# MITIBMxGraph/SALIENT_plusplus

Hardware: AMD Instinct MI355X
Metric: sampled_edges_per_sec (higher is better)
Workload: dtype int64/fp16-copy

## Files before the change

salient_plusplus_amd/csrc/sampler.hip:

```cpp
#include "spp_internal.h"

#include <hipcub/hipcub.hpp>

#include <algorithm>
#include <chrono>
#include <cstdlib>
#include <cstring>
#include <vector>

#include <map>
#include <memory>
#include <mutex>
#include <tuple>

#include "fp8_body.hip.h"
#include "gather_body.hip.h"
#include "partition_common.hip.h"

#ifndef SPP_TILE_NT
#define SPP_TILE_NT 1024
#endif
#include "mt19937.hip.h"
#include "sampler_internal.h"

// ... 788 lines not shown
  for (int u = 0; u < kScatterEPT; ++u) {
    const int64_t p = base + u * kTileNT + threadIdx.x;
    v[u] = cval[p < pcap ? p : pcap - 1];
  }
  if (base >= E || err0) return;
  bool ok[kScatterEPT];
#pragma unroll
  for (int u = 0; u < kScatterEPT; ++u) {
    ok[u] = base + u * kTileNT + threadIdx.x < E;
    v[u] = (int32_t)((uint32_t)v[u] & idmask);
  }
  for (int b = threadIdx.x; b < nbk; b += kTileNT) cur[b] = 0;
  __syncthreads();
#pragma unroll
  for (int u = 0; u < kScatterEPT; ++u)
    if (ok[u]) atomicAdd(&cur[bucket_of((uint32_t)v[u], cb_log2)], 1);
  __syncthreads();
  {
    const int per = (nbk + kTileNT - 1) / kTileNT;
    const int b0 = threadIdx.x * per;
    int32_t c[kMaxBuckets / kTileNT], sum = 0;
#pragma unroll
    for (int k = 0; k < kMaxBuckets / kTileNT; ++k) {
      c[k] = (k < per && b0 + k < nbk) ? cur[b0 + k] : 0;
      sum += c[k];
    }
    int32_t tot;
    int32_t off = block_exclusive_scan<int32_t, kTileNT>(sum, lscan, &tot);
#pragma unroll
    for (int k = 0; k < kMaxBuckets / kTileNT; ++k) {
      if (k < per && b0 + k < nbk) {
        const int32_t g = c[k] ? __hip_atomic_fetch_add(bfill + b0 + k, c[k], __ATOMIC_RELAXED, __HIP_MEMORY_SCOPE_AGENT) : 0;
        cur[b0 + k] = off;
        delta[b0 + k] = g - off;
        off += c[k];
      }
    }
  }
  __syncthreads();
#pragma unroll
  for (int u = 0; u < kScatterEPT; ++u) {
    if (!ok[u]) continue;
    const uint32_t c = (uint32_t)v[u];
    const uint32_t b = bucket_of(c, cb_log2);
    const int32_t slot = atomicAdd(&cur[b], 1);
    const int32_t li = u * kTileNT + threadIdx.x;
    snode[slot] = c;
    sidx[slot] = (uint16_t)li;
    const int32_t rel = slot + delta[b];
    if (rel < bcap) {
      if (!tiled) inv[base + li] = (uint32_t)((int32_t)b * bcap + rel);
    } else {
      const int32_t j = __hip_atomic_fetch_add(G(s.ovfc) + h, 1, __ATOMIC_RELAXED, __HIP_MEMORY_SCOPE_AGENT);
      inv[base + (tiled ? slot : li)] = (uint32_t)(region + j);
      bpairs[(int64_t)region + j] = ((unsigned long long)c << 32) | (uint32_t)(base + li);
    }
  }
  __syncthreads();
  const int32_t n_tile = (int32_t)((E - base) < kScatterTile ? (E - base) : kScatterTile);
  SPP_GLOBAL uint16_t* tidx = G(s.tidx);
  for (int k = threadIdx.x; k < n_tile; k += kTileNT) {
    const uint32_t c = snode[k];
    const int32_t b = (int32_t)bucket_of(c, cb_log2);
    const int32_t rel = k + delta[b];
    if (rel < bcap) {
      bpairs[(int64_t)b * bcap + rel] = ((unsigned long long)c << 32) | (uint32_t)(base + sidx[k]);
      if (tiled) inv[base + k] = (uint32_t)(b * bcap + rel);
    }
    if (tiled) tidx[base + k] = sidx[k];
  }
}

__device__ __forceinline__ int32_t first_rank(const SlotPtrs& s, uint32_t q) {
  const uint32_t w = q >> 6;
  const RankWord rw = s.fwords[w];
  return s.fsum[q >> 8] + (int32_t)rw.pre + __popcll(rw.bits & ((1ull << (q & 63)) - 1ull));
}

template <int NS, bool kFlat = false>
__global__ __launch_bounds__(kNT) __attribute__((amdgpu_waves_per_eu(NS <= 3072 ? 6 : 1))) void k_bucket_dedup(const SlotPtrs* __restrict__ slots, GroupGrid gg,
                                                       int32_t hop_word, DedupGeom g, int32_t bcap, int32_t region) {
  SPP_GROUP_BLOCK(gg);
  const int32_t h = hop_word & 0xff, cb_log2 = (hop_word >> 8) & 0xff, hop_flags = hop_word >> 16;
  const int32_t last_hop = hop_flags & 1;
  const bool no_preread = hop_flags & 2;
  __shared__ unsigned long long tab[NS];
  __shared__ int32_t fkc[kMaxFinePerCoarse];
  __shared__ int32_t fnew[kMaxFinePerCoarse];
  __shared__ int ovf;
  const SlotPtrs& s = slots[gg.first_slot + by_];
  const SPP_GLOBAL SlotState* st = G(s.st);
  const SPP_GLOBAL unsigned long long* bpairs = G(s.bpairs);
  SPP_GLOBAL unsigned long long* known = G(s.known);
  SPP_GLOBAL int32_t* kcount = G(s.kcount);
  const SPP_GLOBAL RankWord* fwords = G(s.fwords);
  const SPP_GLOBAL int32_t* fsum = G(s.fsum);
  SPP_GLOBAL uint32_t* res = G(s.res);
  const int32_t b = bx_;
  const int32_t shift = g.nb_log2 - cb_log2;
  const int32_t nf = 1 << shift;
  const int32_t fb0 = b << shift;
  const int32_t err0 = st->error;
  const uint32_t T = (uint32_t)st->cnt[h];
  const uint32_t Tprev = h > 0 ? (uint32_t)st->cnt[h - 1] : 0u;
  const int32_t fill = __builtin_amdgcn_readfirstlane(G(s.bfill)[b]);
  const int32_t e0 = b * bcap, e1 = e0 + (fill < bcap ? fill : bcap);
  const bool spill = fill > bcap;
  for (int i = threadIdx.x; i < nf; i += kNT) {
    fkc[i] = kcount[fb0 + i];
    fnew[i] = 0;
  }
  const int lane = threadIdx.x & (kWave - 1);
  unsigned long long kpre[4];
  if constexpr (!kFlat) {
    const int lf0 = threadIdx.x / kWave;
    const SPP_GLOBAL unsigned long long* kl0 = known + (int64_t)(fb0 + (lf0 < nf ? lf0 : 0)) * g.kcap;
#pragma unroll
    for (int u = 0; u < 4; ++u) kpre[u] = kl0[lane + u * kWave];
  }
  if (err0) return;
  const bool work = e1 > e0;
  unsigned long long pr[kDedupRegs];
#pragma unroll
  for (int u = 0; u < kDedupRegs; ++u) {
    const int i = e0 + u * kNT + threadIdx.x;
    const unsigned long long v = bpairs[i < e1 ? i : 0];
    pr[u] = i < e1 ? v : kEmptySlot;
  }
  if (work)
    for (int i = threadIdx.x; i < NS; i += kNT) tab[i] = kEmptySlot;
  if (threadIdx.x == 0) ovf = 0;
  __syncthreads();
  if constexpr (kFlat) {
    __shared__ int32_t fpre[kMaxFinePerCoarse + 1];
    if (threadIdx.x < kWave) {
      const int32_t c = (int)threadIdx.x < nf ? fkc[threadIdx.x] : 0;
      const int32_t inc = wave_inclusive_scan(c);
      if ((int)threadIdx.x < nf) fpre[threadIdx.x + 1] = inc;
      if (threadIdx.x == 0) fpre[0] = 0;
    }
    __syncthreads();
    const int32_t K = fpre[nf];
    for (int j0 = threadIdx.x; j0 < K; j0 += 4 * kNT) {
      unsigned long long e[4];
      uint32_t q[4];
      RankWord rw[4];
      int32_t fs[4];
      SPP_GLOBAL unsigned long long* at[4];
#pragma unroll
      for (int u = 0; u < 4; ++u) {
// ... 55 lines not shown
        const bool pend = e[u] != kEmptySlot && (val & kPending);
        q[u] = pend ? (val & ~kPending) : 0u;
        rw[u] = load_rank_word(fwords, q[u] >> 6);
        fs[u] = fsum[q[u] >> 8];
      }
#pragma unroll
      for (int u = 0; u < 4; ++u) {
        if (e[u] == kEmptySlot) continue;
        uint32_t val = (uint32_t)e[u];
        if (val & kPending) {
          val = Tprev + (uint32_t)(fs[u] + (int32_t)rw[u].pre + __popcll(rw[u].bits & ((1ull << (q[u] & 63)) - 1ull)));
          e[u] = (e[u] & 0xffffffff00000000ull) | val;
          kl[i0 + u * kWave] = e[u];
        }
        if (work) lds_upsert<true, NS, false>(tab, (uint32_t)(e[u] >> 32), val, &ovf);
      }
    }
  }
  if (!work) return;
  __syncthreads();
#pragma unroll
  for (int u = 0; u < kDedupRegs; ++u)
    if (pr[u] != kEmptySlot) {
      if (no_preread) lds_upsert<false, NS, false>(tab, (uint32_t)(pr[u] >> 32), T + (uint32_t)pr[u], &ovf);
      else lds_upsert<false, NS>(tab, (uint32_t)(pr[u] >> 32), T + (uint32_t)pr[u], &ovf);
    }
  for (int i0 = e0 + kDedupRegs * kNT + threadIdx.x; i0 < e1; i0 += 4 * kNT) {
    unsigned long long q[4];
#pragma unroll
    for (int u = 0; u < 4; ++u) {
      const int i = i0 + u * kNT;
      const unsigned long long v = bpairs[i < e1 ? i : e0];
      q[u] = i < e1 ? v : kEmptySlot;
    }
#pragma unroll
    for (int u = 0; u < 4; ++u)
      if (q[u] != kEmptySlot) lds_upsert<false, NS, false>(tab, (uint32_t)(q[u] >> 32), T + (uint32_t)q[u], &ovf);
  }
  if (spill) {
    const int32_t n_ovf = G(s.ovfc)[h];
    for (int i = threadIdx.x; i < n_ovf; i += kNT) {
      const unsigned long long q = bpairs[(int64_t)region + i];
      if ((int32_t)bucket_of((uint32_t)(q >> 32), cb_log2) == b) lds_upsert<false, NS, false>(tab, (uint32_t)(q >> 32), T + (uint32_t)q, &ovf);
    }
  }
  __syncthreads();
  if (ovf) {
    if (threadIdx.x == 0) atomicOr(&s.st->error, kErrBucketCap);
    return;
  }
  auto resolve = [&](unsigned long long pair, int i) {
    const uint32_t key = (uint32_t)(pair >> 32), p = (uint32_t)pair;
    const uint32_t val = lds_find<NS>(tab, key);
    res[i] = val;
    if (val == T + p && !last_hop) {
      const int32_t lf = (int32_t)bucket_of(key, g.nb_log2) - fb0;
      const int j = fkc[lf] + atomicAdd(&fnew[lf], 1);
      if (j < g.kcap) known[(int64_t)(fb0 + lf) * g.kcap + j] = ((unsigned long long)key << 32) | kPending | p;
      else ovf = 1;
    }
  };
#pragma unroll
  for (int u = 0; u < kDedupRegs; ++u)
    if (pr[u] != kEmptySlot) resolve(pr[u], e0 + u * kNT + threadIdx.x);
  for (int i = e0 + kDedupRegs * kNT + threadIdx.x; i < e1; i += kNT) resolve(bpairs[i], i);
  if (spill) {
    const int32_t n_ovf = G(s.ovfc)[h];
    for (int i = threadIdx.x; i < n_ovf; i += kNT) {
      const unsigned long long q = bpairs[(int64_t)region + i];
      if ((int32_t)bucket_of((uint32_t)(q >> 32), cb_log2) == b) resolve(q, region + i);
    }
  }
  __syncthreads();
  if (threadIdx.x == 0) G(s.bfill)[b] = 0;
  if (threadIdx.x == 0 && ovf) atomicOr(&s.st->error, kErrBucketCap);
  for (int i = threadIdx.x; i < nf; i += kNT) {
    const int32_t room = g.kcap - fkc[i];
    kcount[fb0 + i] = fkc[i] + (fnew[i] < room ? fnew[i] : room);
  }
}

constexpr int kFlagNT = kNT;
#ifndef SPP_FLAG_ROUNDS
#define SPP_FLAG_ROUNDS 4
#endif
constexpr int kFlagRounds = SPP_FLAG_ROUNDS;
constexpr int kFlagSpan = kFlagNT * kFlagRounds;
static_assert(kFlagNT == 256, "a round of the workgroup is one rank block");

__device__ int32_t scan_block_sums_acquire(int32_t* a, int32_t n, int32_t* lds) {
  int32_t carry = 0;
  for (int32_t base = 0; base < n; base += kFlagNT) {
    const int32_t i = base + threadIdx.x;
    const int32_t v = (i < n) ? acquire_i32(&a[i]) : 0;
    int32_t tot;
    const int32_t ex = block_exclusive_scan<int32_t, kFlagNT>(v, lds, &tot);
    if (i < n) a[i] = carry + ex;
    carry += tot;
    __syncthreads();
  }
  return carry;
}

__global__ __launch_bounds__(kFlagNT) void k_hop_flag(const SlotPtrs* __restrict__ slots, GroupGrid gg, int32_t h,
                                                       int32_t f, int32_t ucap, int64_t pcap) {
  SPP_GROUP_BLOCK(gg);
  __shared__ int32_t wcnt[kFlagRounds][kFlagNT / kWave];
  __shared__ int32_t lscan[kFlagNT / kWave + 1];
  __shared__ int is_last;
  const SlotPtrs& s = slots[gg.first_slot + by_];
  SPP_GLOBAL SlotState* st = G(s.st);
  const SPP_GLOBAL uint32_t* inv = G(s.inv);
  const SPP_GLOBAL uint32_t* res = G(s.res);
  SPP_GLOBAL uint32_t* evals = G(s.evals);
  const int64_t base = (int64_t)bx_ * kFlagSpan;
  const int32_t err0 = st->error;
  const int32_t E = st->E[h];
  const uint32_t T = (uint32_t)st->cnt[h];
  uint32_t slot[kFlagRounds];
#pragma unroll
  for (int r = 0; r < kFlagRounds; ++r) {
    const int64_t p = base + r * kFlagNT + threadIdx.x;
    slot[r] = inv[p < pcap ? p : pcap - 1];
  }
  if (err0) {
    if (bx_ == 0 && threadIdx.x == 0) {
      st->cnt[h + 1] = (int32_t)T;
      st->dbase[h + 1] = st->dbase[h];
    }
    return;
  }
  const int32_t nwg = E > 0 ? (E + kFlagSpan - 1) / kFlagSpan : 1;
  if ((int32_t)bx_ >= nwg) return;
  const int wid = threadIdx.x / kWave, lane = threadIdx.x & (kWave - 1);
  uint32_t val[kFlagRounds];
#pragma unroll
  for (int r = 0; r < kFlagRounds; ++r) {
    const int64_t p = base + r * kFlagNT + threadIdx.x;
    val[r] = res[p < E ? slot[r] : 0u];
  }
  unsigned long long bits[kFlagRounds];
#pragma unroll
  for (int r = 0; r < kFlagRounds; ++r) {
    const int64_t p = base + r * kFlagNT + threadIdx.x;
    bool flag = false;
    if (p < E) {
      evals[p] = val[r];
      flag = (val[r] == T + (uint32_t)p);
    }
    bits[r] = __ballot(flag);
    if (lane == 0) wcnt[r][wid] = __popcll(bits[r]);
  }
  __syncthreads();
  if (lane == 0) {
#pragma unroll
    for (int r = 0; r < kFlagRounds; ++r) {
      int32_t pre = 0;
      for (int k = 0; k < wid; ++k) pre += wcnt[r][k];
      const int64_t blk = (int64_t)bx_ * kFlagRounds + r;
      s.fwords[blk * (kFlagNT / kWave) + wid] = RankWord{bits[r], (uint32_t)pre, 0u};
      if (wid == kFlagNT / kWave - 1)
        __hip_atomic_store(&s.fsum[blk], pre + wcnt[r][wid], __ATOMIC_RELAXED, __HIP_MEMORY_SCOPE_AGENT);
    }
  }
  asm volatile("s_waitcnt vmcnt(0)" ::: "memory");
  __syncthreads();
  if (threadIdx.x == 0) is_last = take_ticket_is_last(s.ctr, nwg) ? 1 : 0;
  __syncthreads();
  if (!is_last) return;
  const int32_t nblk = (E + 255) / 256;
  const int32_t nnew = scan_block_sums_acquire(s.fsum, nblk, lscan);
  if (threadIdx.x == 0) {
    const int32_t U = st->cnt[h] + nnew;
    st->cnt[h + 1] = U;
    st->dbase[h + 1] = st->dbase[h] + (int64_t)(f > 0 ? f : 0) * st->nsmp[h];
    if (U > ucap) atomicOr(&s.st->error, kErrNodeCap);
  }
}

constexpr int kFlagTileRounds = kScatterTile / kFlagNT;
__global__ __launch_bounds__(kFlagNT) void k_hop_flag_tiled(const SlotPtrs* __restrict__ slots, GroupGrid gg, int32_t h,
                                                             int32_t f, int32_t ucap, int64_t pcap) {
  SPP_GROUP_BLOCK(gg);
  __shared__ uint32_t vals[kScatterTile];
  __shared__ unsigned long long wbits[kFlagTileRounds * (kFlagNT / kWave)];
  __shared__ int32_t wcnt[kFlagTileRounds * (kFlagNT / kWave)];
  __shared__ int32_t lscan[kFlagNT / kWave + 1];
  static_assert(kFlagTileRounds * (kFlagNT / kWave) <= kFlagNT, "one thread per bitmap word of the tile");
  __shared__ int is_last;
  const SlotPtrs& s = slots[gg.first_slot + by_];
  SPP_GLOBAL SlotState* st = G(s.st);
  const SPP_GLOBAL uint32_t* inv = G(s.inv);
  const SPP_GLOBAL uint16_t* tidx = G(s.tidx);
  const SPP_GLOBAL uint32_t* res = G(s.res);
  SPP_GLOBAL uint32_t* evals = G(s.evals);
  const int64_t base = (int64_t)bx_ * kScatterTile;
  const int32_t err0 = st->error;
  const int32_t E = st->E[h];
  const uint32_t T = (uint32_t)st->cnt[h];
  if (err0) {
// ... 751 lines not shown
    uint32_t mask[8] = {0, 0, 0, 0, 0, 0, 0, 0};
    const char* lay = getenv("SPP_CU_MASK_LAYOUT");
    if (lay && !strcmp(lay, "blocked")) {
      const int per_xcd = (ncu + 7) / 8;
      int left = ncu;
      for (int x = 0; x < 8 && left > 0; ++x)
        for (int k = 0; k < per_xcd && k < 32 && left > 0; ++k, --left) mask[x] |= 1u << k;
    } else {
      for (int k = 0; k < ncu; ++k) mask[k >> 5] |= 1u << (k & 31);
    }
    if (hipExtStreamCreateWithCUMask(st, 8, mask) == hipSuccess) return hipSuccess;
    (void)hipGetLastError();
  }
  return prio ? hipStreamCreateWithPriority(st, hipStreamNonBlocking, prio) : hipStreamCreateWithFlags(st, hipStreamNonBlocking);
}

static std::mutex g_col32_mu;
static std::map<std::tuple<const void*, int64_t, int, int64_t, int>, std::weak_ptr<Col32>> g_col32;

struct RowStubs {
  stub4* p = nullptr;
  int device = 0;
  bool from_col32 = false;
  ~RowStubs() {
    (void)hipSetDevice(device);
    if (p) (void)hipFree(p);
  }
};
static std::map<std::tuple<const void*, const void*, int64_t, int, int64_t, const void*>, std::weak_ptr<RowStubs>> g_stubs;

struct SlotHost {
  SlotPtrs p{};
  hipEvent_t done = nullptr;
  hipEvent_t exported = nullptr;
  hipEvent_t wait_on = nullptr;
  SlotState* host_state = nullptr;
  bool sampled = false;
  bool waited = false;
  int64_t ecap_dyn[SPP_MAX_HOPS];
  int64_t etmp_cap = 0;
  void* cub_tmp = nullptr;
  size_t cub_tmp_bytes = 0;
};

struct ResolvedOpts {
  int col32 = 1;
  int deg_tags = 1;
  int row_stubs = -1;
  int rng_arena = -1;
  int64_t rng_arena_words = 0;
  int fuse = 1;
  int64_t fuse_max_edges = 262144;
  bool flag_tiled = true, rows_coalesced = true, dedup_preread = false;
};

struct HopPlan {
  bool self_prefix = false;
  bool fused = false;
  bool flag_tiled = false;
  bool rows_coal = false;
  unsigned row_lds = 0;
  unsigned lds_fused = 0;
  int64_t tile_cap = 0;
};

struct spp_sampler {
  spp_sampler_cfg cfg{};
  ResolvedOpts opt{};
  HopPlan plan[SPP_MAX_HOPS];
  int rng_arena_decision = -1;
  double col32_ms = 0, stubs_ms = 0;
  hipEvent_t arena_t0 = nullptr, arena_t1 = nullptr;
  double rng_arena_ms = 0;
  bool arena_timed = false;
  int64_t tcap[SPP_MAX_HOPS + 1];
  int64_t ecap[SPP_MAX_HOPS];
  int64_t dcap = 0;
  bool generic[SPP_MAX_HOPS];
  bool any_generic = false;
  DedupGeom geom{};
  int cb_log2[SPP_MAX_HOPS];
  int lds_log2 = 12;
  int64_t bytes = 0;
  std::vector<SlotHost> slots;
  std::vector<void*> allocs;
  hipStream_t deliver_stream = nullptr;
  hipStream_t comm_stream = nullptr;
  hipStream_t work_streams[kMaxWorkStreams] = {};
  SlotPtrs* d_slots = nullptr;
  SlotState* d_states = nullptr;
  SlotState* h_states = nullptr;
  int32_t* counts = nullptr;
  int64_t counts_per_slot = 0;
  std::shared_ptr<Col32> col32_owner;
  int32_t* col32 = nullptr;
  std::shared_ptr<RowStubs> stubs_owner;
  const stub4* stubs = nullptr;
  int idbits = 32;
  uint32_t idmask = 0xffffffffu;
  uint32_t tag_cap = 0;
  bool use_tags = false;
  uint32_t* rng_arena = nullptr;
  int64_t rng_arena_words = 0;
  int64_t rng_arena_stride = 0;
  std::vector<uint32_t> rng_arena_seeds;
  uint32_t* rng_arena_seeds_dev = nullptr;
  int64_t rng_arena_seeds_cap = 0;
  hipEvent_t rng_arena_ready = nullptr;
  hipEvent_t inputs_ready = nullptr;
  unsigned long long* cache_bits = nullptr;
  hipEvent_t cache_bits_ready = nullptr;
  std::unique_ptr<Worker> workers[2];
// ... 29 lines not shown
              cfg->num_hops, SPP_MAX_HOPS);
  SPP_REQUIRE(cfg->rowptr_dev && (cfg->col_dev || cfg->nnz == 0), "spp_sampler_create: NULL graph");
  SPP_REQUIRE(cfg->num_nodes > 0 && cfg->num_nodes < (1ll << 31), "spp_sampler_create: num_nodes %lld must be < 2^31",
              (long long)cfg->num_nodes);
  SPP_REQUIRE(cfg->max_batch > 0 && cfg->num_slots > 0, "spp_sampler_create: max_batch and num_slots must be > 0");
  const spp_partition_cfg& pc = cfg->part;
  SPP_REQUIRE(pc.num_parts >= 0 && pc.num_parts <= SPP_MAX_PARTS, "spp_sampler_create: num_parts %d not in [0,%d]",
              pc.num_parts, SPP_MAX_PARTS);
  if (pc.num_parts > 0) {
    SPP_REQUIRE(pc.rank >= 0 && pc.rank < pc.num_parts, "spp_sampler_create: rank %d out of [0,%d)", pc.rank,
                pc.num_parts);
    SPP_REQUIRE(!pc.use_cache || (pc.cache_map_dev && pc.cache_map_len > 0),
                "spp_sampler_create: use_cache without a cache map");
    for (int m = 0; m < pc.num_parts; ++m)
      SPP_REQUIRE(pc.offsets[m] <= pc.offsets[m + 1], "spp_sampler_create: partition offsets must be non-decreasing");
    SPP_REQUIRE(pc.offsets[0] <= 0 && pc.offsets[pc.num_parts] >= cfg->num_nodes,
                "spp_sampler_create: partition offsets [%lld,%lld) do not cover the %lld nodes",
                (long long)pc.offsets[0], (long long)pc.offsets[pc.num_parts], (long long)cfg->num_nodes);
  }
  int ndev = spp_device_count();
  SPP_REQUIRE(ndev > 0, "spp_sampler_create: no HIP device available (the on-GPU sampler has no CPU fallback)");
  SPP_HIP_TRY(hipSetDevice(cfg->device));

  auto* s = new spp_sampler();
  s->cfg = *cfg;
  if (const char* e = getenv("SPP_XCD_AFFINITY")) s->xcd_affinity = atoi(e) != 0;
  {
    const spp_sampler_opts& o = cfg->opts;
    auto env_int = [](const char* name, long long dflt) -> long long {
      const char* e = getenv(name);
      return e && *e ? atoll(e) : dflt;
    };
    auto sw = [&](int32_t field, const char* name, int dflt) -> int {
      if (field) return field > 0 ? 1 : 0;
      return env_int(name, dflt) != 0 ? 1 : 0;
    };
    ResolvedOpts& r = s->opt;
    r.col32 = sw(o.col32, "SPP_COL32", 1);
    r.deg_tags = sw(o.deg_tags, "SPP_DEG_TAGS", 1);
    if (o.row_stubs) r.row_stubs = o.row_stubs > 0 ? 1 : 0;
    else {
      const long long m = env_int("SPP_ROW_STUBS", -1);
      r.row_stubs = m < 0 ? -1 : (m > 0 ? 1 : 0);
    }
    const bool env_budget = getenv("SPP_RNG_ARENA_MB") != nullptr;
    const long long mb = o.rng_arena_mb > 0 ? o.rng_arena_mb : env_int("SPP_RNG_ARENA_MB", 16384);
    r.rng_arena_words = (mb < 0 ? 0 : mb) * (int64_t)(1 << 20) / 4;
    if (o.rng_arena) r.rng_arena = o.rng_arena > 0 ? 1 : 0;
    else r.rng_arena = (o.rng_arena_mb > 0 || env_budget) ? 1 : -1;
    if (o.fuse_scatter) r.fuse = o.fuse_scatter < 0 ? 0 : std::min(o.fuse_scatter, 2);
    else r.fuse = (int)std::max<long long>(0, std::min<long long>(2, env_int("SPP_FUSE_SCATTER", 1)));
    r.fuse_max_edges = o.fuse_max_edges > 0 ? o.fuse_max_edges : env_int("SPP_FUSE_MAX_EDGES", 262144);
    r.flag_tiled = sw(o.flag_tiled, "SPP_FLAG_TILED", 1) != 0;
    r.rows_coalesced = sw(o.rows_coalesced, "SPP_ROWS_COALESCED", 1) != 0;
    r.dedup_preread = sw(o.dedup_preread, "SPP_DEDUP_PREREAD", 0) != 0;
  }
  const int H = cfg->num_hops;
  const int64_t node_bound = cfg->num_nodes + cfg->max_batch;
  s->tcap[0] = cfg->max_batch;
  int64_t etmp = 1;
  for (int h = 0; h < H; ++h) {
    const int64_t f = cfg->sizes[h];
    s->generic[h] = (f < 0 || f > kFastMaxFanout);
    s->any_generic |= s->generic[h];
    if (f >= 0) {
      s->ecap[h] = s->tcap[h] * f;
      s->tcap[h + 1] = std::min(s->tcap[h] * (1 + f), node_bound);
      s->dcap += f * s->tcap[h];
    } else {
      s->ecap[h] = cfg->opts.initial_edge_cap > 0 ? cfg->opts.initial_edge_cap
                                                  : std::min<int64_t>(std::max<int64_t>(cfg->nnz, 1), 1 << 22);
      s->tcap[h + 1] = node_bound;
    }
    etmp = std::max(etmp, s->ecap[h]);
  }
  const int64_t ucap = s->tcap[H];
  if (ucap + etmp >= (1ll << 31) || region_for(etmp) + etmp >= (1ll << 31)) {
    set_error("spp_sampler_create: batch too large for 32-bit positions");
    delete s;
    return SPP_ERR_INVALID;
  }
  static const int64_t bucket_nodes = [] {
    const char* e = getenv("SPP_DEDUP_BUCKET");
    const int64_t v = e ? atoll(e) : 1536;
    return v < 64 ? 64 : v;
  }();
  int nb_log2 = 0;
  while (nb_log2 < kMaxBucketsLog2 && (ucap >> nb_log2) > bucket_nodes) ++nb_log2;
  s->geom.nb_log2 = nb_log2;
  s->geom.nb = 1 << nb_log2;
  const int64_t per_bucket = (ucap + s->geom.nb - 1) / s->geom.nb;
  s->geom.kcap = (int32_t)std::min<int64_t>(per_bucket + per_bucket / 2 + 256, 0x7fffffff);
  s->lds_log2 = per_bucket > 6144 ? 14 : (per_bucket > 1536 ? 13 : (per_bucket > 820 ? 12 : 11));
  for (int h = 0; h < H; ++h) {
    int c = std::max(0, nb_log2 - kMaxFineLog2);
    while (c < nb_log2 && (s->tcap[h + 1] >> c) > bucket_nodes) ++c;
    s->cb_log2[h] = c;
  }
  const int nb = s->geom.nb;
  int64_t tmax = 0;
  for (int h = 0; h < H; ++h) tmax = std::max(tmax, s->tcap[h]);
  const int64_t nblk_max = std::max(ceil_div(tmax, kNT), ceil_div(etmp, kNT)) + 1;
  const int nslots = cfg->num_slots;
  if (pc.num_parts > 0) {
    s->part.P = pc.num_parts;
    s->part.rank = pc.rank;
// ... 173 lines not shown
          }
        }
      }
    }
    if (rc == SPP_OK && c && c->p) {
      s->stubs_owner = c;
      s->stubs = c->p;
      s->bytes += (int64_t)need;
      bool fits = s->col32 && c->from_col32 && s->idbits < 32 && !cfg->replace;
      for (int h = 1; h < H && fits; ++h) fits = cfg->sizes[h] >= 0 && (uint64_t)cfg->sizes[h] < s->col32_owner->cap;
      if (fits) {
        s->use_tags = true;
        s->tag_cap = s->col32_owner->cap;
      }
    }
  }
  if (rc == SPP_OK) {
    const int need = (int)(sizeof(int32_t) * 2 * kMaxBuckets + (sizeof(uint32_t) + sizeof(uint16_t)) * kScatterTile);
    int have = 0;
    (void)hipDeviceGetAttribute(&have, hipDeviceAttributeMaxSharedMemoryPerBlock, cfg->device);
    if (have < need + 1024 ||
        hipFuncSetAttribute(reinterpret_cast<const void*>(&k_bucket_scatter), hipFuncAttributeMaxDynamicSharedMemorySize,
                            need) != hipSuccess) {
      set_error("spp_sampler_create: the device offers %d bytes of LDS per workgroup, k_bucket_scatter needs %d "
                "(this library targets gfx950)", have, need + 1024);
      (void)hipGetLastError();
      rc = SPP_ERR_HIP;
    }
  }
  if (rc == SPP_OK) {
    int lds_limit = 0;
    (void)hipDeviceGetAttribute(&lds_limit, hipDeviceAttributeMaxSharedMemoryPerBlock, cfg->device);
    hipFuncAttributes fattr{};
    const void* fused_fn = reinterpret_cast<const void*>(&k_hop_pick<false, int32_t, true, true, true>);
    const int lds_static = hipFuncGetAttributes(&fattr, fused_fn) == hipSuccess ? (int)fattr.sharedSizeBytes : 8 * 1024;
    (void)hipGetLastError();
    unsigned lds_fused_max = 0;
    for (int h = 0; h < H; ++h) {
      HopPlan& pl = s->plan[h];
      const int32_t f = (int32_t)cfg->sizes[h];
      const int32_t fc = std::max<int32_t>(1, std::min<int32_t>(f, kFastMaxFanout));
      const int64_t gt = std::max<int64_t>(1, ceil_div(s->tcap[h], kNT));
      pl.row_lds = (unsigned)(sizeof(int32_t) * kNT * (size_t)fc);
      pl.self_prefix = !s->generic[h] && gt <= 2048;
      const unsigned nbk = 1u << s->cb_log2[h];
      pl.tile_cap = (int64_t)kNT * fc;
      pl.lds_fused = pl.row_lds + (unsigned)(sizeof(int32_t) * 2 * nbk + (sizeof(uint32_t) + sizeof(uint16_t)) * (size_t)pl.tile_cap);
      pl.fused = !s->generic[h] && pl.self_prefix && s->col32 && s->stubs && s->use_tags && s->opt.fuse != 0 && f >= 1 &&
                 nbk <= (unsigned)kMaxBuckets && pl.lds_fused <= 64u * 1024u &&
                 (int64_t)pl.lds_fused + lds_static <= (int64_t)lds_limit &&
                 (s->opt.fuse >= 2 || (pl.tile_cap >= 8 * (int64_t)nbk && s->ecap[h] <= s->opt.fuse_max_edges));
      if (pl.fused) lds_fused_max = std::max(lds_fused_max, pl.lds_fused);
      pl.flag_tiled = s->opt.flag_tiled && !pl.fused && !s->generic[h];
      pl.rows_coal = !s->generic[h] && s->opt.rows_coalesced && f >= 1 && f <= 28;
    }
    if (lds_fused_max > 0) {
      static unsigned fused_lds_attr = 0;
      std::lock_guard<std::mutex> lk(g_col32_mu);
      bool ok = lds_fused_max <= fused_lds_attr;
      if (!ok && hipFuncSetAttribute(fused_fn, hipFuncAttributeMaxDynamicSharedMemorySize, (int)lds_fused_max) == hipSuccess) {
        fused_lds_attr = lds_fused_max;
        ok = true;
      }
      (void)hipGetLastError();
      if (!ok)
        for (int h = 0; h < H; ++h)
          if (s->plan[h].fused && s->plan[h].lds_fused > 64u * 1024u) {
            s->plan[h].fused = false;
            s->plan[h].flag_tiled = s->opt.flag_tiled;
          }
    }
  }
  if (rc == SPP_OK && create_data_stream(&s->deliver_stream, false) != hipSuccess) {
    set_error("spp_sampler_create: stream creation failed");
    rc = SPP_ERR_HIP;
  }
  if (rc == SPP_OK) {
    std::vector<SlotPtrs> tmp((size_t)nslots);
    for (int i = 0; i < nslots; ++i) tmp[(size_t)i] = s->slots[(size_t)i].p;
    if (hipMemcpy(s->d_slots, tmp.data(), sizeof(SlotPtrs) * (size_t)nslots, hipMemcpyHostToDevice) != hipSuccess) {
      set_error("spp_sampler_create: upload of the slot table failed");
      rc = SPP_ERR_HIP;
    }
  }
  if (rc != SPP_OK) {
    spp_sampler_destroy(s);
    return rc;
  }
  *out = s;
  return SPP_OK;
}

extern "C" void spp_sampler_destroy(spp_sampler* s) {
  if (!s) return;
  s->workers[0].reset();
  s->workers[1].reset();
  (void)hipSetDevice(s->cfg.device);
  (void)hipDeviceSynchronize();
  for (auto& sl : s->slots) {
    if (sl.done) (void)hipEventDestroy(sl.done);
    if (sl.exported) (void)hipEventDestroy(sl.exported);
    if (sl.p.cval) (void)hipFree(sl.p.cval);
    if (sl.p.bpairs) (void)hipFree(sl.p.bpairs);
    if (sl.p.evals) (void)hipFree(sl.p.evals);
    if (sl.p.inv) (void)hipFree(sl.p.inv);
    if (sl.p.tidx) (void)hipFree(sl.p.tidx);
    if (sl.p.res) (void)hipFree(sl.p.res);
    if (sl.p.fwords) (void)hipFree(sl.p.fwords);
    if (sl.cub_tmp) (void)hipFree(sl.cub_tmp);
  }
  if (s->rng_arena) (void)hipFree(s->rng_arena);
  if (s->rng_arena_seeds_dev) (void)hipFree(s->rng_arena_seeds_dev);
  if (s->rng_arena_ready) (void)hipEventDestroy(s->rng_arena_ready);
  if (s->arena_t0) (void)hipEventDestroy(s->arena_t0);
  if (s->arena_t1) (void)hipEventDestroy(s->arena_t1);
  if (s->inputs_ready) (void)hipEventDestroy(s->inputs_ready);
  if (s->cache_bits_ready) (void)hipEventDestroy(s->cache_bits_ready);
  if (s->cache_bits) (void)hipFree(s->cache_bits);
  if (s->h_states) (void)hipHostFree(s->h_states);
  if (s->deliver_stream) (void)hipStreamDestroy(s->deliver_stream);
  for (auto st : s->work_streams)
    if (st) (void)hipStreamDestroy(st);
  if (s->comm_stream) (void)hipStreamDestroy(s->comm_stream);
  for (auto& d : s->dargs_host)
    if (d) (void)hipHostFree(d);
  for (auto& d : s->dargs_dev)
    if (d) (void)hipFree(d);
  for (auto& xb : s->xbuf) {
    if (xb.cnt_dev) (void)hipFree(xb.cnt_dev);
    if (xb.cnt_host) (void)hipHostFree(xb.cnt_host);
    if (xb.cnt_ready) (void)hipEventDestroy(xb.cnt_ready);
    if (xb.rows_done) (void)hipEventDestroy(xb.rows_done);
    if (xb.send_ids) (void)hipFree(xb.send_ids);
    if (xb.recv_ids) (void)hipFree(xb.recv_ids);
    if (xb.send_rows) (void)hipFree(xb.send_rows);
    if (xb.recv_rows) (void)hipFree(xb.recv_rows);
  }
  for (void* a : s->allocs) (void)hipFree(a);
  delete s;
}

extern "C" int64_t spp_sampler_workspace_bytes(const spp_sampler* s) { return s ? s->bytes : 0; }

extern "C" void* spp_sampler_deliver_stream(spp_sampler* s) { return s ? (void*)s->deliver_stream : nullptr; }

extern "C" spp_status spp_sampler_get_cfg(const spp_sampler* s, spp_sampler_cfg* out) {
  SPP_REQUIRE(s && out, "spp_sampler_get_cfg: NULL argument");
  *out = s->cfg;
  return SPP_OK;
}

extern "C" spp_status spp_sampler_get_info(spp_sampler* s, spp_sampler_info* out) {
  SPP_REQUIRE(s && out, "spp_sampler_get_info: NULL argument");
  memset(out, 0, sizeof(*out));
  const int H = s->cfg.num_hops;
  out->col32 = s->col32 ? 1 : 0;
  out->deg_tags = s->use_tags ? 1 : 0;
  out->row_stubs = s->stubs ? 1 : 0;
  out->rng_arena = s->rng_arena_decision;
  out->idbits = s->idbits;
  out->tag_cap = (int32_t)s->tag_cap;
  out->num_hops = H;
  out->dedup_buckets_log2 = s->geom.nb_log2;
  out->dedup_table_slots = s->lds_log2 == 11 ? 2048 : (s->lds_log2 == 12 ? SPP_DEDUP_SLOTS12 : (s->lds_log2 == 13 ? 8192 : 16384));
  for (int h = 0; h < H; ++h) {
    out->generic[h] = s->generic[h] ? 1 : 0;
    out->fused_pick[h] = s->plan[h].fused ? 1 : 0;
    out->flag_tiled[h] = s->plan[h].flag_tiled ? 1 : 0;
    out->rows_coalesced[h] = s->plan[h].rows_coal ? 1 : 0;
    out->bucket_log2[h] = s->cb_log2[h];
  }
  if (s->arena_timed) {
    (void)hipSetDevice(s->cfg.device);
    float ms = 0.f;
    if (hipEventSynchronize(s->arena_t1) == hipSuccess && hipEventElapsedTime(&ms, s->arena_t0, s->arena_t1) == hipSuccess)
      s->rng_arena_ms = ms;
    (void)hipGetLastError();
    s->arena_timed = false;
  }
  out->col32_ms = s->col32_ms;
  out->row_stubs_ms = s->stubs_ms;
  out->rng_arena_ms = s->rng_arena_ms;
  out->col32_bytes = s->col32 ? (int64_t)sizeof(int32_t) * (s->cfg.nnz + 16) : 0;
  out->row_stubs_bytes = s->stubs ? (int64_t)sizeof(int32_t) * kStubInts * s->cfg.num_nodes : 0;
  out->rng_arena_bytes = 4 * s->rng_arena_words;
  out->rng_arena_batches = (int64_t)s->rng_arena_seeds.size();
  return SPP_OK;
}

static spp_status grow_edge_scratch(spp_sampler* s, int slot, int h, int64_t need, hipStream_t st) {
  SlotHost& sl = s->slots[(size_t)slot];
  bool changed = false;
  if (need > sl.etmp_cap) {
    int64_t cap = std::max(need, sl.etmp_cap * 2);
    RankWord* old_fwords = sl.p.fwords;
    int32_t* old_fsum = sl.p.fsum;
    const int64_t old_cap = sl.etmp_cap;
    (void)hipFree(sl.p.cval); (void)hipFree(sl.p.bpairs); (void)hipFree(sl.p.evals);
    (void)hipFree(sl.p.inv); (void)hipFree(sl.p.res); (void)hipFree(sl.p.tidx);
    sl.p.tidx = nullptr;
    sl.p.cval = nullptr; sl.p.bpairs = nullptr; sl.p.evals = nullptr; sl.p.fwords = nullptr;
    sl.p.inv = nullptr; sl.p.res = nullptr;
    SPP_HIP_TRY(hipMalloc((void**)&sl.p.cval, sizeof(int32_t) * (size_t)cap));
    SPP_REQUIRE(region_for(cap) + cap < (1ll << 31), "spp_sampler: a hop of %lld edges exceeds 32-bit bucket positions", (long long)need);
    const size_t n_bucketed = (size_t)(region_for(cap) + cap);
    SPP_HIP_TRY(hipMalloc((void**)&sl.p.bpairs, sizeof(unsigned long long) * n_bucketed));
    SPP_HIP_TRY(hipMalloc((void**)&sl.p.evals, sizeof(uint32_t) * (size_t)cap));
    SPP_HIP_TRY(hipMalloc((void**)&sl.p.inv, sizeof(uint32_t) * (size_t)cap));
    SPP_HIP_TRY(hipMalloc((void**)&sl.p.tidx, sizeof(uint16_t) * (size_t)cap));
    SPP_HIP_TRY(hipMalloc((void**)&sl.p.res, sizeof(uint32_t) * n_bucketed));
    SPP_HIP_TRY(hipMalloc((void**)&sl.p.fwords, rank_bytes(cap)));
    sl.p.fsum = reinterpret_cast<int32_t*>(reinterpret_cast<char*>(sl.p.fwords) + rank_off_fsum(cap));
    SPP_HIP_TRY(hipMemcpy(sl.p.fwords, old_fwords, 16 * (size_t)rank_words(old_cap), hipMemcpyDeviceToDevice));
    SPP_HIP_TRY(hipMemcpy(sl.p.fsum, old_fsum, 4 * (size_t)rank_blocks(old_cap), hipMemcpyDeviceToDevice));
    (void)hipFree(old_fwords);
    s->bytes += 48 * (cap - sl.etmp_cap) + (int64_t)rank_bytes(cap) - (int64_t)rank_bytes(sl.etmp_cap);
    sl.etmp_cap = cap;
    changed = true;
  }
  if (need > sl.ecap_dyn[h]) {
    int64_t cap = std::max(need, sl.ecap_dyn[h] * 2);
// ... 176 lines not shown
    const int32_t cb = s->cb_log2[h];
    const unsigned nbk = 1u << cb;
    const int64_t pcap = std::max<int64_t>(1, s->generic[h] ? 0 : s->ecap[h]);
    const bool fused = pl.fused;
    const int64_t tile_cap = pl.tile_cap;
    const unsigned lds_fused = pl.lds_fused;
    if (!s->generic[h]) {
      if (fused) {
        FuseArgs fa{cb, bucket_cap(pcap, nbk), (int32_t)region_for(lead.etmp_cap), idmask, (int32_t)(row_lds / sizeof(int32_t)), (int32_t)tile_cap};
        const unsigned lds = lds_fused;
        hipLaunchKernelGGL((k_hop_pick<false, int32_t, true, true, true>), dim3((gt) * gy), dim3(kNT), lds, st, s->d_slots, GG(gt),
                           col32, stubs, h, f, replace, self_prefix, ecap_dev, s->dcap, (int32_t)s->tcap[h], pick_mask, fa);
      } else if (col32 && stubs && s->use_tags)
        hipLaunchKernelGGL((k_hop_pick<false, int32_t, true, true>), dim3((gt) * gy), dim3(kNT), row_lds, st, s->d_slots, GG(gt),
                           col32, stubs, h, f, replace, self_prefix, ecap_dev, s->dcap, (int32_t)s->tcap[h], pick_mask, fa_plain);
      else if (col32 && stubs)
        hipLaunchKernelGGL((k_hop_pick<false, int32_t, true>), dim3((gt) * gy), dim3(kNT), row_lds, st, s->d_slots, GG(gt),
                           col32, stubs, h, f, replace, self_prefix, ecap_dev, s->dcap, (int32_t)s->tcap[h], pick_mask, fa_plain);
      else if (col32)
        hipLaunchKernelGGL((k_hop_pick<false, int32_t, false>), dim3((gt) * gy), dim3(kNT), row_lds, st, s->d_slots, GG(gt),
                           col32, stubs, h, f, replace, self_prefix, ecap_dev, s->dcap, (int32_t)s->tcap[h], pick_mask, fa_plain);
      else if (stubs)
        hipLaunchKernelGGL((k_hop_pick<false, int64_t, true>), dim3((gt) * gy), dim3(kNT), row_lds, st, s->d_slots, GG(gt),
                           col, stubs, h, f, replace, self_prefix, ecap_dev, s->dcap, (int32_t)s->tcap[h], pick_mask, fa_plain);
      else
        hipLaunchKernelGGL((k_hop_pick<false, int64_t, false>), dim3((gt) * gy), dim3(kNT), row_lds, st, s->d_slots, GG(gt),
                           col, stubs, h, f, replace, self_prefix, ecap_dev, s->dcap, (int32_t)s->tcap[h], pick_mask, fa_plain);
      ge = (unsigned)std::max<int64_t>(1, ceil_div(s->ecap[h], kNT));
    } else {
      SPP_HIP_TRY(hipMemcpyAsync(lead.host_state, lead.p.st, sizeof(SlotState), hipMemcpyDeviceToHost, st));
      SPP_HIP_TRY(hipStreamSynchronize(st));
      const int64_t E = lead.host_state->E[h];
      if (lead.host_state->error) break;
      SPP_TRY(grow_edge_scratch(s, first_slot, h, E, st));
      ge = (unsigned)std::max<int64_t>(1, ceil_div(E, kNT));
      hipLaunchKernelGGL((k_hop_pick<true, int64_t, false>), dim3((gt) * gy), dim3(kNT), sizeof(int32_t) * kNT, st, s->d_slots,
                         GG(gt), col, stubs, h, f, replace, 0, ecap_dev, s->dcap, (int32_t)s->tcap[h], pick_mask, fa_plain);
      if (col32)
        hipLaunchKernelGGL(k_hop_expand_generic<int32_t>, dim3((ge) * gy), dim3(kNT), 0, st, s->d_slots, GG(ge), col32,
                           h, f, replace, idmask);
      else
        hipLaunchKernelGGL(k_hop_expand_generic<int64_t>, dim3((ge) * gy), dim3(kNT), 0, st, s->d_slots, GG(ge), col,
                           h, f, replace, idmask);
    }
    const int32_t region = (int32_t)region_for(lead.etmp_cap);
    const bool dedup_preread = s->opt.dedup_preread;
    const int32_t last = ((h == H - 1) ? 1 : 0) | (!dedup_preread ? 2 : 0);
    const int32_t hop_word = h | (s->cb_log2[h] << 8) | (last << 16);
    const int64_t pcap_h = s->generic[h] ? std::max<int64_t>(1, lead.host_state->E[h]) : pcap;
    const unsigned gsc = (unsigned)std::max<int64_t>(1, ceil_div((int64_t)ge * kNT, kScatterTile));
    const unsigned sc_lds = (unsigned)(sizeof(int32_t) * 2 * nbk + (sizeof(uint32_t) + sizeof(uint16_t)) * kScatterTile);
    const int32_t bcap = bucket_cap(pcap_h, nbk);
    const bool flag_tiled = pl.flag_tiled;
    if (!fused)
      hipLaunchKernelGGL(k_bucket_scatter, dim3((gsc) * gy), dim3(kTileNT), sc_lds, st, s->d_slots, GG(gsc), h, cb, bcap, region, pcap_h, idmask,
                         flag_tiled ? 1 : 0);
    static const unsigned dedup_pad = [] { const char* e = getenv("SPP_WHATIF_DEDUP_LDS_PAD"); return e ? (unsigned)atoi(e) : 0u; }();
    const unsigned dpad = (h == H - 1) ? dedup_pad : 0u;
    static const bool dedup_flat_on = [] { const char* e = getenv("SPP_DEDUP_FLAT"); return !e || atoi(e) != 0; }();
    const bool flat = dedup_flat_on && (geom.nb_log2 - cb) > 2;
    if (s->lds_log2 == 11 && flat)
      hipLaunchKernelGGL((k_bucket_dedup<2048, true>), dim3((nbk) * gy), dim3(kNT), dpad, st, s->d_slots, GG(nbk), hop_word, geom, bcap, region);
    else if (s->lds_log2 == 12 && flat)
      hipLaunchKernelGGL((k_bucket_dedup<SPP_DEDUP_SLOTS12, true>), dim3((nbk) * gy), dim3(kNT), dpad, st, s->d_slots, GG(nbk), hop_word, geom, bcap, region);
    else if (s->lds_log2 == 11)
      hipLaunchKernelGGL(k_bucket_dedup<2048>, dim3((nbk) * gy), dim3(kNT), dpad, st, s->d_slots, GG(nbk), hop_word, geom, bcap, region);
    else if (s->lds_log2 == 12)
      hipLaunchKernelGGL(k_bucket_dedup<SPP_DEDUP_SLOTS12>, dim3((nbk) * gy), dim3(kNT), dpad, st, s->d_slots, GG(nbk), hop_word, geom, bcap, region);
    else if (s->lds_log2 == 13)
      hipLaunchKernelGGL(k_bucket_dedup<8192>, dim3((nbk) * gy), dim3(kNT), 0, st, s->d_slots, GG(nbk), hop_word, geom, bcap, region);
    else
      hipLaunchKernelGGL(k_bucket_dedup<16384>, dim3((nbk) * gy), dim3(kNT), 0, st, s->d_slots, GG(nbk), hop_word, geom, bcap, region);
    const unsigned gflag = (unsigned)std::max<int64_t>(1, ceil_div((int64_t)ge * kNT, kFlagSpan));
    for (int rep = 0; rep < dup.flag; ++rep) {
      if (flag_tiled)
        hipLaunchKernelGGL(k_hop_flag_tiled, dim3((gsc) * gy), dim3(kFlagNT), 0, st, s->d_slots, GG(gsc), h, f,
                           (int32_t)s->tcap[H], pcap_h);
      else
        hipLaunchKernelGGL(k_hop_flag, dim3((gflag) * gy), dim3(kFlagNT), 0, st, s->d_slots, GG(gflag), h, f,
                           (int32_t)s->tcap[H], pcap_h);
    }
    if (!s->generic[h]) {
      const int32_t run_cap = (int32_t)(kNT * std::max<int32_t>(1, std::min<int32_t>(f, kFastMaxFanout)));
      for (int rep = 0; rep < dup.rows; ++rep) {
        if (pl.rows_coal)
          hipLaunchKernelGGL(k_hop_rows_coalesced, dim3((gt) * gy), dim3(kNT), (unsigned)(8 * run_cap), st, s->d_slots, GG(gt), h,
                             idmask, row_idbits, (int32_t)s->tcap[h], pcap_h, run_cap);
        else
          hipLaunchKernelGGL(k_hop_rows, dim3((gt) * gy), dim3(kNT), row_lds, st, s->d_slots, GG(gt), h, idmask, row_idbits,
                             (int32_t)s->tcap[h], pcap_h);
      }
    } else {
      const int64_t E = lead.host_state->E[h];
      const int32_t T = lead.host_state->cnt[h];
      if (E > 0) {
        hipLaunchKernelGGL(k_hop_lids_generic, dim3((ge) * gy), dim3(kNT), 0, st, s->d_slots, GG(ge), h);
        size_t need = 0;
        SPP_HIP_TRY(hipcub::DeviceSegmentedRadixSort::SortKeys(nullptr, need, lead.p.cval, lead.p.out_col[h], (int)E, T,
                                                               lead.p.out_rowptr[h], lead.p.out_rowptr[h] + 1, 0, 32,
                                                               st));
        if (need > lead.cub_tmp_bytes) {
          SPP_HIP_TRY(hipStreamSynchronize(st));
          if (lead.cub_tmp) (void)hipFree(lead.cub_tmp);
          lead.cub_tmp = nullptr;
          SPP_HIP_TRY(hipMalloc(&lead.cub_tmp, need));
          lead.cub_tmp_bytes = need;
        }
        size_t have = lead.cub_tmp_bytes;
        SPP_HIP_TRY(hipcub::DeviceSegmentedRadixSort::SortKeys(lead.cub_tmp, have, lead.p.cval, lead.p.out_col[h],
                                                               (int)E, T, lead.p.out_rowptr[h],
                                                               lead.p.out_rowptr[h] + 1, 0, 32, st));
      }
    }
  }
  if (s->part.P > 0) {
    const unsigned gu = (unsigned)std::max<int64_t>(1, ceil_div(s->tcap[H], kPartSpan));
    hipLaunchKernelGGL(k_gpart_hist, dim3((gu) * gy), dim3(kNT), 0, st, s->d_slots, GG(gu), H, s->part, (int32_t)s->tcap[H]);
    hipLaunchKernelGGL(k_gpart_scan, dim3((1) * gy), dim3(kScanNT), 0, st, s->d_slots, GG(1), H, s->part);
    hipLaunchKernelGGL(k_gpart_scatter, dim3((gu) * gy), dim3(kNT), 0, st, s->d_slots, GG(gu), H, s->part, (int32_t)s->tcap[H]);
  }
  prof_end(SPP_PROF_CHAIN, prof, st);
  SPP_HIP_TRY(hipGetLastError());
  SPP_HIP_TRY(hipMemcpyAsync(lead.host_state, lead.p.st, sizeof(SlotState) * (size_t)n, hipMemcpyDeviceToHost, st));
  SPP_HIP_TRY(hipEventRecord(lead.done, st));
  for (int i = 0; i < n; ++i) {
    SlotHost& sl = s->slots[(size_t)(first_slot + i)];
    sl.wait_on = lead.done;
    sl.sampled = true;
    sl.waited = false;
  }
  return SPP_OK;
}
// ... 458 lines not shown
```

Baseline: 8.514 billion.

## Store dedup results by edge position on last hop, skipping inv indirection

On the last hop with tiled flagging, the dedup kernel now writes each resolved value straight to evals at its original edge position rather than to a bucket-ordered res array. The scatter kernel then skips writing the inv and tidx arrays, and a sequential flag kernel variant reads evals directly instead of gathering through inv and res. This is meant to remove the indirect gather and several global writes in exchange for scattered writes from the dedup kernel. A what-if env path that double-writes is also added for experimentation.

```diff
diff --git a/salient_plusplus_amd/csrc/sampler.hip b/salient_plusplus_amd/csrc/sampler.hip
--- a/salient_plusplus_amd/csrc/sampler.hip
+++ b/salient_plusplus_amd/csrc/sampler.hip
@@ -864,7 +864,7 @@
       if (!tiled) inv[base + li] = (uint32_t)((int32_t)b * bcap + rel);
     } else {
       const int32_t j = __hip_atomic_fetch_add(G(s.ovfc) + h, 1, __ATOMIC_RELAXED, __HIP_MEMORY_SCOPE_AGENT);
-      inv[base + (tiled ? slot : li)] = (uint32_t)(region + j);
+      if (tiled != 2) inv[base + (tiled ? slot : li)] = (uint32_t)(region + j);
       bpairs[(int64_t)region + j] = ((unsigned long long)c << 32) | (uint32_t)(base + li);
     }
   }
@@ -877,9 +877,9 @@
     const int32_t rel = k + delta[b];
     if (rel < bcap) {
       bpairs[(int64_t)b * bcap + rel] = ((unsigned long long)c << 32) | (uint32_t)(base + sidx[k]);
-      if (tiled) inv[base + k] = (uint32_t)(b * bcap + rel);
-    }
-    if (tiled) tidx[base + k] = sidx[k];
+      if (tiled == 1) inv[base + k] = (uint32_t)(b * bcap + rel);
+    }
+    if (tiled == 1) tidx[base + k] = sidx[k];
   }
 }
 
@@ -889,7 +889,7 @@
   return s.fsum[q >> 8] + (int32_t)rw.pre + __popcll(rw.bits & ((1ull << (q & 63)) - 1ull));
 }
 
-template <int NS, bool kFlat = false>
+template <int NS, bool kFlat = false, int kPos = 0>
 __global__ __launch_bounds__(kNT) __attribute__((amdgpu_waves_per_eu(NS <= 3072 ? 6 : 1))) void k_bucket_dedup(const SlotPtrs* __restrict__ slots, GroupGrid gg,
                                                        int32_t hop_word, DedupGeom g, int32_t bcap, int32_t region) {
   SPP_GROUP_BLOCK(gg);
@@ -907,7 +907,7 @@
   SPP_GLOBAL int32_t* kcount = G(s.kcount);
   const SPP_GLOBAL RankWord* fwords = G(s.fwords);
   const SPP_GLOBAL int32_t* fsum = G(s.fsum);
-  SPP_GLOBAL uint32_t* res = G(s.res);
+  SPP_GLOBAL uint32_t* res = G(kPos == 2 ? s.evals : s.res);
   const int32_t b = bx_;
   const int32_t shift = g.nb_log2 - cb_log2;
   const int32_t nf = 1 << shift;
@@ -1069,7 +1069,12 @@
   auto resolve = [&](unsigned long long pair, int i) {
     const uint32_t key = (uint32_t)(pair >> 32), p = (uint32_t)pair;
     const uint32_t val = lds_find<NS>(tab, key);
-    res[i] = val;
+    if constexpr (kPos == 2) {
+      res[p] = val;
+    } else {
+      res[i] = val;
+      if constexpr (kPos == 1) G(s.evals)[p] = val;
+    }
     if (val == T + p && !last_hop) {
       const int32_t lf = (int32_t)bucket_of(key, g.nb_log2) - fb0;
       const int j = fkc[lf] + atomicAdd(&fnew[lf], 1);
@@ -1119,6 +1124,7 @@
   return carry;
 }
 
+template <bool kSeq = false>
 __global__ __launch_bounds__(kFlagNT) void k_hop_flag(const SlotPtrs* __restrict__ slots, GroupGrid gg, int32_t h,
                                                        int32_t f, int32_t ucap, int64_t pcap) {
   SPP_GROUP_BLOCK(gg);
@@ -1138,7 +1144,7 @@
 #pragma unroll
   for (int r = 0; r < kFlagRounds; ++r) {
     const int64_t p = base + r * kFlagNT + threadIdx.x;
-    slot[r] = inv[p < pcap ? p : pcap - 1];
+    slot[r] = (kSeq ? evals : inv)[p < pcap ? p : pcap - 1];
   }
   if (err0) {
     if (bx_ == 0 && threadIdx.x == 0) {
@@ -1154,7 +1160,7 @@
 #pragma unroll
   for (int r = 0; r < kFlagRounds; ++r) {
     const int64_t p = base + r * kFlagNT + threadIdx.x;
-    val[r] = res[p < E ? slot[r] : 0u];
+    val[r] = kSeq ? slot[r] : res[p < E ? slot[r] : 0u];
   }
   unsigned long long bits[kFlagRounds];
 #pragma unroll
@@ -1162,7 +1168,7 @@
     const int64_t p = base + r * kFlagNT + threadIdx.x;
     bool flag = false;
     if (p < E) {
-      evals[p] = val[r];
+      if (!kSeq) evals[p] = val[r];
       flag = (val[r] == T + (uint32_t)p);
     }
     bits[r] = __ballot(flag);
@@ -2020,12 +2026,14 @@
   int fuse = 1;
   int64_t fuse_max_edges = 262144;
   bool flag_tiled = true, rows_coalesced = true, dedup_preread = false;
+  bool pos_store = true;
 };
 
 struct HopPlan {
   bool self_prefix = false;
   bool fused = false;
   bool flag_tiled = false;
+  bool pos_store = false;
   bool rows_coal = false;
   unsigned row_lds = 0;
   unsigned lds_fused = 0;
@@ -2161,6 +2169,7 @@
     else r.fuse = (int)std::max<long long>(0, std::min<long long>(2, env_int("SPP_FUSE_SCATTER", 1)));
     r.fuse_max_edges = o.fuse_max_edges > 0 ? o.fuse_max_edges : env_int("SPP_FUSE_MAX_EDGES", 262144);
     r.flag_tiled = sw(o.flag_tiled, "SPP_FLAG_TILED", 1) != 0;
+    r.pos_store = (o.flag_tiled ? (long long)o.flag_tiled : env_int("SPP_FLAG_TILED", 1)) < 2;
     r.rows_coalesced = sw(o.rows_coalesced, "SPP_ROWS_COALESCED", 1) != 0;
     r.dedup_preread = sw(o.dedup_preread, "SPP_DEDUP_PREREAD", 0) != 0;
   }
@@ -2440,6 +2449,7 @@
                  (s->opt.fuse >= 2 || (pl.tile_cap >= 8 * (int64_t)nbk && s->ecap[h] <= s->opt.fuse_max_edges));
       if (pl.fused) lds_fused_max = std::max(lds_fused_max, pl.lds_fused);
       pl.flag_tiled = s->opt.flag_tiled && !pl.fused && !s->generic[h];
+      pl.pos_store = pl.flag_tiled && s->opt.pos_store && h == H - 1;
       pl.rows_coal = !s->generic[h] && s->opt.rows_coalesced && f >= 1 && f <= 28;
     }
     if (lds_fused_max > 0) {
@@ -2456,6 +2466,7 @@
           if (s->plan[h].fused && s->plan[h].lds_fused > 64u * 1024u) {
             s->plan[h].fused = false;
             s->plan[h].flag_tiled = s->opt.flag_tiled;
+            s->plan[h].pos_store = s->opt.flag_tiled && s->opt.pos_store && h == H - 1;
           }
     }
   }
@@ -2554,7 +2565,7 @@
   for (int h = 0; h < H; ++h) {
     out->generic[h] = s->generic[h] ? 1 : 0;
     out->fused_pick[h] = s->plan[h].fused ? 1 : 0;
-    out->flag_tiled[h] = s->plan[h].flag_tiled ? 1 : 0;
+    out->flag_tiled[h] = s->plan[h].flag_tiled ? ((h == s->cfg.num_hops - 1 && !s->plan[h].pos_store) ? 2 : 1) : 0;
     out->rows_coalesced[h] = s->plan[h].rows_coal ? 1 : 0;
     out->bucket_log2[h] = s->cb_log2[h];
   }
@@ -2837,32 +2848,43 @@
     const unsigned sc_lds = (unsigned)(sizeof(int32_t) * 2 * nbk + (sizeof(uint32_t) + sizeof(uint16_t)) * kScatterTile);
     const int32_t bcap = bucket_cap(pcap_h, nbk);
     const bool flag_tiled = pl.flag_tiled;
+    const bool pos_store = pl.pos_store;
+    static const bool whatif_pos = [] { const char* e = getenv("SPP_WHATIF_DEDUP_POS_STORE"); return e && atoi(e) != 0; }();
     if (!fused)
       hipLaunchKernelGGL(k_bucket_scatter, dim3((gsc) * gy), dim3(kTileNT), sc_lds, st, s->d_slots, GG(gsc), h, cb, bcap, region, pcap_h, idmask,
-                         flag_tiled ? 1 : 0);
+                         pos_store ? 2 : flag_tiled ? 1 : 0);
     static const unsigned dedup_pad = [] { const char* e = getenv("SPP_WHATIF_DEDUP_LDS_PAD"); return e ? (unsigned)atoi(e) : 0u; }();
     const unsigned dpad = (h == H - 1) ? dedup_pad : 0u;
     static const bool dedup_flat_on = [] { const char* e = getenv("SPP_DEDUP_FLAT"); return !e || atoi(e) != 0; }();
     const bool flat = dedup_flat_on && (geom.nb_log2 - cb) > 2;
-    if (s->lds_log2 == 11 && flat)
-      hipLaunchKernelGGL((k_bucket_dedup<2048, true>), dim3((nbk) * gy), dim3(kNT), dpad, st, s->d_slots, GG(nbk), hop_word, geom, bcap, region);
-    else if (s->lds_log2 == 12 && flat)
-      hipLaunchKernelGGL((k_bucket_dedup<SPP_DEDUP_SLOTS12, true>), dim3((nbk) * gy), dim3(kNT), dpad, st, s->d_slots, GG(nbk), hop_word, geom, bcap, region);
-    else if (s->lds_log2 == 11)
-      hipLaunchKernelGGL(k_bucket_dedup<2048>, dim3((nbk) * gy), dim3(kNT), dpad, st, s->d_slots, GG(nbk), hop_word, geom, bcap, region);
-    else if (s->lds_log2 == 12)
-      hipLaunchKernelGGL(k_bucket_dedup<SPP_DEDUP_SLOTS12>, dim3((nbk) * gy), dim3(kNT), dpad, st, s->d_slots, GG(nbk), hop_word, geom, bcap, region);
-    else if (s->lds_log2 == 13)
-      hipLaunchKernelGGL(k_bucket_dedup<8192>, dim3((nbk) * gy), dim3(kNT), 0, st, s->d_slots, GG(nbk), hop_word, geom, bcap, region);
-    else
-      hipLaunchKernelGGL(k_bucket_dedup<16384>, dim3((nbk) * gy), dim3(kNT), 0, st, s->d_slots, GG(nbk), hop_word, geom, bcap, region);
+    auto dedup = [&](auto fn, unsigned lds) {
+      hipLaunchKernelGGL(fn, dim3((nbk) * gy), dim3(kNT), lds, st, s->d_slots, GG(nbk), hop_word, geom, bcap, region);
+    };
+    if (pos_store) {
+      if (s->lds_log2 == 11 && flat) dedup(k_bucket_dedup<2048, true, 2>, dpad);
+      else if (s->lds_log2 == 12 && flat) dedup(k_bucket_dedup<SPP_DEDUP_SLOTS12, true, 2>, dpad);
+      else if (s->lds_log2 == 11) dedup(k_bucket_dedup<2048, false, 2>, dpad);
+      else if (s->lds_log2 == 12) dedup(k_bucket_dedup<SPP_DEDUP_SLOTS12, false, 2>, dpad);
+      else if (s->lds_log2 == 13) dedup(k_bucket_dedup<8192, false, 2>, 0u);
+      else dedup(k_bucket_dedup<16384, false, 2>, 0u);
+    } else if (whatif_pos && flag_tiled && h == H - 1 && s->lds_log2 == 12 && !flat)
+      dedup(k_bucket_dedup<SPP_DEDUP_SLOTS12, false, 1>, dpad);
+    else if (s->lds_log2 == 11 && flat) dedup(k_bucket_dedup<2048, true>, dpad);
+    else if (s->lds_log2 == 12 && flat) dedup(k_bucket_dedup<SPP_DEDUP_SLOTS12, true>, dpad);
+    else if (s->lds_log2 == 11) dedup(k_bucket_dedup<2048>, dpad);
+    else if (s->lds_log2 == 12) dedup(k_bucket_dedup<SPP_DEDUP_SLOTS12>, dpad);
+    else if (s->lds_log2 == 13) dedup(k_bucket_dedup<8192>, 0u);
+    else dedup(k_bucket_dedup<16384>, 0u);
     const unsigned gflag = (unsigned)std::max<int64_t>(1, ceil_div((int64_t)ge * kNT, kFlagSpan));
     for (int rep = 0; rep < dup.flag; ++rep) {
-      if (flag_tiled)
+      if (pos_store)
+        hipLaunchKernelGGL(k_hop_flag<true>, dim3((gflag) * gy), dim3(kFlagNT), 0, st, s->d_slots, GG(gflag), h, f,
+                           (int32_t)s->tcap[H], pcap_h);
+      else if (flag_tiled)
         hipLaunchKernelGGL(k_hop_flag_tiled, dim3((gsc) * gy), dim3(kFlagNT), 0, st, s->d_slots, GG(gsc), h, f,
                            (int32_t)s->tcap[H], pcap_h);
       else
-        hipLaunchKernelGGL(k_hop_flag, dim3((gflag) * gy), dim3(kFlagNT), 0, st, s->d_slots, GG(gflag), h, f,
+        hipLaunchKernelGGL(k_hop_flag<false>, dim3((gflag) * gy), dim3(kFlagNT), 0, st, s->d_slots, GG(gflag), h, f,
                            (int32_t)s->tcap[H], pcap_h);
     }
     if (!s->generic[h]) {
```

After: 8.241 billion. 3.2% lower.
